# NVlabs/DREAM

Hardware: AMD Instinct MI355X
Metric: frames/s DREAM-vgg-q 400x400 b=128 inference (higher is better)
Workload: dtype f32

## Files before the change

### dream_amd/csrc/conv_first.hip

```cpp
#include <dream_cdna4.h>
#include "common.h"
#include "../../include/dream_hip.h"

namespace {
constexpr int FT = 16;
constexpr int FPW = FT + 4;
constexpr int FPH = FT + 2;
constexpr int FMAXC = 4;
constexpr int FPAIRS = FPH - 1;
constexpr int FPLANE = FPAIRS * FPW * 2;


struct FirstParams {
    const float *x;
    const float *w;
    const float *bias;
    float *y;
    unsigned *amax_out;
    int B, H, W, Cin, Cout;
    int tiles_x, tiles_y;
    int relu;
};

__global__ void __launch_bounds__(256) conv3x3_first_kernel(const FirstParams p) {
    DREAM_DYNAMIC_LDS(float, smem);
    const int tid = threadIdx.x, lane = tid & 63, wave = wave_index();
    int t = blockIdx.x;
    const int tix = t % p.tiles_x;
    t /= p.tiles_x;
    const int tiy = t % p.tiles_y;
    const int b = t / p.tiles_y;
    const int y0 = tiy * FT, x0 = tix * FT;
    const int cout = blockIdx.y * 64 + lane;

    const int npatch = p.Cin * FPH * FPW;
    for (int idx = tid; idx < npatch; idx += 256) {
        const int c = idx / (FPH * FPW);
        const int rem = idx - c * (FPH * FPW);
        const int py = rem / FPW, px = rem - py * FPW;
        const int gy = y0 - 1 + py, gx = x0 - 1 + px;
        float v = 0.0f;
        if (px < FT + 2 && gy >= 0 && gy < p.H && gx >= 0 && gx < p.W)
            v = p.x[(((size_t)b * p.Cin + c) * p.H + gy) * p.W + gx];
        if (py < FPAIRS) smem[c * FPLANE + (py * FPW + px) * 2] = v;
        if (py > 0) smem[c * FPLANE + ((py - 1) * FPW + px) * 2 + 1] = v;
    }
    float wr[FMAXC * 9];
#pragma unroll
    for (int i = 0; i < FMAXC * 9; ++i) wr[i] = (i < p.Cin * 9) ? p.w[(size_t)cout * p.Cin * 9 + i] : 0.0f;
    const float bv = p.bias ? p.bias[cout] : 0.0f;
    __syncthreads();

    float amax = 0.0f;
    for (int g = 0; g < 8; ++g) {
        const int row = wave * 4 + 2 * (g >> 2), xg = (g & 3) * 4;
        f32x2 acc[4];
#pragma unroll
        for (int i = 0; i < 4; ++i) acc[i] = f32x2{bv, bv};
#pragma unroll
        for (int c = 0; c < FMAXC; ++c) {
            if (c < p.Cin) {
#pragma unroll
                for (int ky = 0; ky < 3; ++ky) {
                    const float *src = smem + c * FPLANE + ((row + ky) * FPW + xg) * 2;
                    const f32x4 q0 = *(const f32x4 *)src, q1 = *(const f32x4 *)(src + 4), q2 = *(const f32x4 *)(src + 8);
                    const f32x2 v[6] = {{q0[0], q0[1]}, {q0[2], q0[3]}, {q1[0], q1[1]}, {q1[2], q1[3]}, {q2[0], q2[1]}, {q2[2], q2[3]}};
#pragma unroll
                    for (int kx = 0; kx < 3; ++kx) {
                        const float wv = wr[c * 9 + ky * 3 + kx];
                        const f32x2 w2 = {wv, wv};
#pragma unroll
                        for (int i = 0; i < 4; ++i) acc[i] = __builtin_elementwise_fma(v[i + kx], w2, acc[i]);
                    }
                }
            }
        }
        if (p.relu) {
#pragma unroll
            for (int i = 0; i < 4; ++i) acc[i] = f32x2{fmaxf(acc[i][0], 0.0f), fmaxf(acc[i][1], 0.0f)};
        }
        const int ox = x0 + xg;
#pragma unroll
        for (int h = 0; h < 2; ++h) {
            const int oy = y0 + row + h;
            if (oy < p.H) {
                float *dst = p.y + (((size_t)b * p.H + oy) * p.W + ox) * p.Cout + cout;
#pragma unroll
                for (int i = 0; i < 4; ++i)
                    if (ox + i < p.W) { dst[(size_t)i * p.Cout] = acc[i][h]; amax = fmaxf(amax, fabsf(acc[i][h])); }
            }
        }
    }
    if (p.amax_out != nullptr) publish_amax(p.amax_out, amax);
}
}

static int first_impl(const float *x_nchw, const float *w_oihw, const float *bias, float *y_nhwc, int B, int H, int W,
                      int Cin, int Cout, int relu, void *stream, unsigned *amax_out) {
    DREAM_REQUIRE(x_nchw && w_oihw && y_nhwc, "null pointer");
    DREAM_REQUIRE(B > 0 && H > 0 && W > 0, "bad shape");
    DREAM_REQUIRE(Cin >= 1 && Cin <= FMAXC, "first conv supports Cin <= %d (got %d)", FMAXC, Cin);
    DREAM_REQUIRE(Cout % 64 == 0, "first conv needs Cout %% 64 == 0 (got %d)", Cout);
    FirstParams p;
    p.x = x_nchw; p.w = w_oihw; p.bias = bias; p.y = y_nhwc; p.amax_out = amax_out;
    p.B = B; p.H = H; p.W = W; p.Cin = Cin; p.Cout = Cout; p.relu = relu;
    p.tiles_x = ceil_div(W, FT); p.tiles_y = ceil_div(H, FT);
    const size_t lds = (size_t)Cin * FPLANE * sizeof(float);
    const dim3 grid((unsigned)((size_t)B * p.tiles_x * p.tiles_y), (unsigned)(Cout / 64));
    hipLaunchKernelGGL(conv3x3_first_kernel, grid, dim3(256), lds, (hipStream_t)stream, p);
    DREAM_LAUNCH_OK();
    return 0;
}

extern "C" int dream_conv3x3_first_nchw_f32(const float *x_nchw, const float *w_oihw, const float *bias,
                                            float *y_nhwc, int B, int H, int W, int Cin, int Cout,
                                            int relu, void *stream) {
    return first_impl(x_nchw, w_oihw, bias, y_nhwc, B, H, W, Cin, Cout, relu, stream, nullptr);
}
extern "C" int dream_conv3x3_first_nchw_amax_f32(const float *x_nchw, const float *w_oihw, const float *bias,
                                                 float *y_nhwc, unsigned *amax_out, int B, int H, int W, int Cin,
                                                 int Cout, int relu, void *stream) {
    return first_impl(x_nchw, w_oihw, bias, y_nhwc, B, H, W, Cin, Cout, relu, stream, amax_out);
}
```

### dream_amd/csrc/conv_wino4.hip

```cpp
#include <type_traits>
#include <stdlib.h>
#include <dream_cdna4.h>
#include "common.h"
#include "pack_device.h"
#include "../../include/dream_hip.h"

#ifndef DREAM_W4_DIAG
#define DREAM_W4_DIAG 0
#endif
#ifndef DREAM_W4_STORE
#define DREAM_W4_STORE buffer_store_f32
#endif
#ifndef DREAM_W4_MIDBARRIER
#define DREAM_W4_MIDBARRIER 0
#endif
#ifndef DREAM_W4_STAGGER_N
#define DREAM_W4_STAGGER_N 0
#define DREAM_W4_STAGGER_PCT 0
#endif
#ifndef DREAM_W4_WAUX
#define DREAM_W4_WAUX 0
#endif
#ifndef DREAM_W4_XAUX
#define DREAM_W4_XAUX 0
#endif
#ifndef DREAM_W4_STAG_LX
#define DREAM_W4_STAG_LX 0
#endif
#ifndef DREAM_W4_RUNNING_WOFF
#define DREAM_W4_RUNNING_WOFF 1
#endif
#ifndef DREAM_W4_SETPRIO
#define DREAM_W4_SETPRIO 0
#endif

namespace {

struct Wino4Params {
    const float *x;
    const float *u;
    const float *scale;
    const float *shift;
    const float *residual;
    float *y;
    float *y_full;
    int B, H, W, Cin, Cout, CoutPad;
    int TY, TX;
    int ntiles;
    int nblk, blk_per_xcd;
    unsigned long long magic_tpi, magic_tx;
    int flags;
    int out_scale, out_oy, out_ox;
    int in_scale, in_oy, in_ox;
    int stagger_n, stagger_unit;
    int ymap;
};

constexpr int W4T = 16;
constexpr int W4P = 36;
#ifndef DREAM_W4_RING
#define DREAM_W4_RING 8
#endif
#ifndef DREAM_W4_NARROW_RING
#define DREAM_W4_NARROW_RING 18
#endif
#ifndef DREAM_W4_PAT_RING
#define DREAM_W4_PAT_RING 10
#endif
#ifndef DREAM_W4_PAT_S1OFF
#define DREAM_W4_PAT_S1OFF 8
#endif


template <bool NARROW>
struct W4Cfg {
    static constexpr int NW = NARROW ? 4 : 8;
    static constexpr int K = NARROW ? 8 : 16;
    static constexpr int Q = K / 4;
    static constexpr int KS = K / 4;
    static constexpr int PAD = 16 * NW;
    static constexpr int VPS = NARROW ? W4T * K : W4T * K + 16;
    static constexpr int VB = W4P * VPS;
    static constexpr int SROW = NARROW ? 14 : 25;
    static constexpr int QS = NARROW ? 7 : 6;
    static constexpr int SB = W4T * 6 * SROW * 4;
    static constexpr int RING = NARROW ? DREAM_W4_NARROW_RING : DREAM_W4_RING;
    static constexpr int AHEAD = RING - 2;
    static_assert(72 % RING == 0, "the weight ring must divide two chunks' positions");
    using vec = std::conditional_t<NARROW, f32x2, f32x4>;
};
template <bool NARROW>
DREAM_DEVICE int v4_slot(int q, int t) { return NARROW ? q ^ ((t >> 3) & 1) : q ^ ((t >> 2) & 2); }

DREAM_DEVICE f32x4 fma4(float c, f32x4 a, f32x4 b) {
    f32x4 r;
#pragma unroll
    for (int k = 0; k < 4; ++k) r[k] = __builtin_fmaf(c, a[k], b[k]);
    return r;
}

DREAM_DEVICE f32x4 sub4(f32x4 y, f32x4 x) { return pk_sub4(y, x); }
DREAM_DEVICE f32x4 bt_row(int j, const f32x4 *d) {
    switch (j) {
        case 0: return fma4(-2.0f, d[2], fma4(1.5f, sub4(d[3], d[1]), d[0] + d[4]));
        case 1: return fma4(2.5f, d[3], fma4(0.5f, d[2], sub4(d[4], d[1])));
        case 2: return fma4(0.5f, d[3], fma4(-2.5f, d[2], d[4] + d[1]));
        case 3: return fma4(2.0f, sub4(d[3], d[1]), sub4(d[4], d[2]));
        case 4: return fma4(-0.5f, sub4(d[3], d[1]), sub4(d[4], d[2]));
        default: return fma4(-2.0f, d[3], fma4(1.5f, sub4(d[4], d[2]), d[1] + d[5]));
    }
}

DREAM_DEVICE constexpr bool pat4_row_active(int pat, int i) { return pat == 0 || (((pat - 1) >> 1) == 0 ? i <= 4 : i >= 1); }
DREAM_DEVICE constexpr bool pat4_col_active(int pat, int j) { return pat == 0 || (((pat - 1) & 1) == 0 ? j <= 4 : j >= 1); }
DREAM_DEVICE constexpr bool pat4_active(int pat, int pp) { return pat4_row_active(pat, pp / 6) && pat4_col_active(pat, pp % 6); }
DREAM_DEVICE constexpr int pat4_count(int pat) { return pat == 0 ? 36 : 25; }
struct Pat4Table { int pos[36]; };
constexpr Pat4Table pat4_table(int pat) {
    Pat4Table t = {};
    int n = 0;
    for (int pp = 0; pp < 36; ++pp)
        if (pat4_active(pat, pp)) t.pos[n++] = pp;
    return t;
}
template <int PAT>
struct Pat4 { static constexpr Pat4Table table = pat4_table(PAT); };
#define pat4_pos(PAT, k) (Pat4<PAT>::table.pos[k])

template <int MODE, bool NARROW, int PAT = 0>
__global__ void __launch_bounds__(64 * W4Cfg<NARROW>::NW, 2) conv_wino4_kernel(const Wino4Params p) {
    using C = W4Cfg<NARROW>;
    using vec = typename C::vec;
    constexpr int W4K = C::K, W4NW = C::NW, V4PS = C::VPS, V4B = C::VB, S4ROW = C::SROW;
    constexpr int NPOS = pat4_count(PAT);
    constexpr int W4_RING = PAT ? DREAM_W4_PAT_RING : C::RING, W4_AHEAD = W4_RING - 2;
    static_assert((2 * NPOS) % W4_RING == 0, "the weight ring must divide two chunks' positions");
    DREAM_DYNAMIC_LDS(float, sV);
    const int tid = threadIdx.x;
    const int lane = tid & 63;
    const int wave = wave_index();
    const int item_id = wave * 48 + (lane < 48 ? lane : lane - 16);

    const int xcd = (int)(blockIdx.x & 7), J = (int)(gridDim.x >> 3);
    const int part = p.ymap ? xcd / p.ymap : xcd;
    const int blk_hi = (part + 1) * p.blk_per_xcd;
    const int blk_end = blk_hi < p.nblk ? blk_hi : p.nblk;
    int tb = part * p.blk_per_xcd + (int)(blockIdx.x >> 3);
    if (tb >= blk_end) return;
    const int n0 = (p.ymap ? xcd % p.ymap : (int)blockIdx.y) * (16 * W4NW);
    if (p.stagger_n > 1) {
        const unsigned w = blockIdx.x + blockIdx.y * gridDim.x;
        const int naps = (int)((w * 2654435761u >> 16) % (unsigned)p.stagger_n) * p.stagger_unit;
        for (int i = 0; i < naps; ++i) __builtin_amdgcn_s_sleep(127);
    }
    const int tiles_per_img = p.TY * p.TX;
    const int Si = PAT ? p.in_scale : 1;
    const size_t img_floats = (size_t)(Si * p.H) * (Si * p.W) * p.Cin;

    const int q1 = item_id % C::Q, r1 = (item_id / C::Q) % 6, t1 = (item_id / C::Q) / 6;
    const int s1_off = ((t1 * 6 + r1) * S4ROW + C::QS * q1) * 4;
    const int q2 = item_id % C::Q;
    const int j2 = NARROW ? (item_id >> 3) % 6 : (item_id >> 2) % 6;
    const int t2 = NARROW ? 4 * (item_id / 48) + ((item_id >> 1) & 3) : (item_id >> 2) / 6;
    const int s2_off = ((t2 * 6) * S4ROW + C::QS * q2 + j2) * 4;
    const int v2_off = j2 * V4PS + t2 * W4K + 4 * v4_slot<NARROW>(q2, t2);

    unsigned goff0;
    int item1 = t1 | (r1 << 8) | (q1 << 16);
    auto plan_item = [&](int tile0, int b0) {
        asm volatile("" : "+v"(item1));
        const int t = item1 & 255, r = (item1 >> 8) & 255, q = (item1 >> 16) & 255;
        const int tau = tile0 + t;
        const bool tv = tau < p.ntiles;
        const int b = div_magic40(tau, p.magic_tpi), rem = tau - b * tiles_per_img;
        const int ty = div_magic40(rem, p.magic_tx), tx = rem - ty * p.TX;
        const int gy = 4 * ty - 1 + r, x0 = 4 * tx - 1;
        const bool rok = tv & ((unsigned)gy < (unsigned)p.H);
        goff0 = PAT ? (unsigned)(((((b - b0) * Si * p.H + Si * gy + p.in_oy) * (Si * p.W) + Si * x0 + p.in_ox) * p.Cin + 4 * q) * 4)
                    : (unsigned)(((((b - b0) * p.H + gy) * p.W + x0) * p.Cin + 4 * q) * 4);
        item1 &= 0xffffff;
#pragma unroll
        for (int c = 0; c < 6; ++c) item1 |= (rok & ((unsigned)(x0 + c) < (unsigned)p.W)) ? (1 << (24 + c)) : 0;
    };
    const unsigned px_in = (unsigned)(Si * p.Cin * 4);
    auto item_offset = [&](int c) {
        if (DREAM_W4_DIAG & 16) {
            unsigned o = BUFFER_OOB;
            asm volatile("" : "+v"(o));
            return o;
        }
        return (item1 >> (24 + c)) & 1 ? goff0 + (unsigned)c * px_in : BUFFER_OOB;
    };
    auto block_tile0 = [&](int blk) { return blk < blk_end ? blk * W4T : p.ntiles; };
    auto block_xbuf = [&](int b0) {
        return make_buffer(p.x + (size_t)b0 * img_floats, ((size_t)(p.B - b0) * img_floats) * sizeof(float));
    };

    const int lt = lane & 15, lg = lane >> 4;
    const int a_off = NARROW ? lt * W4K + 4 * v4_slot<NARROW>(lg >> 1, lt) + 2 * (lg & 1) : lt * W4K + 4 * v4_slot<NARROW>(lg, lt);
    const unsigned b_lane = (unsigned)(((wave * 16 + lt) * W4K + C::KS * lg) * 4);
    const unsigned u_pos_stride = (unsigned)(p.CoutPad * W4K * 4);
    const BufferRsrc ubuf = make_buffer(p.u + (size_t)n0 * W4K, ((size_t)((p.Cin / W4K) * W4P + C::AHEAD) * p.CoutPad - (size_t)n0) * W4K * sizeof(float));

    f32x4 acc[W4P];
    const int nchunks = p.Cin / W4K;
    if (DREAM_W4_SETPRIO && wave >= W4NW / 2) __builtin_amdgcn_s_setprio(1);

    vec bq[W4_RING];
    auto load_u = [&](unsigned soff) {
        if constexpr (NARROW) return buffer_load_x2(ubuf, b_lane, soff);
        else return buffer_load_x4_aux<DREAM_W4_WAUX>(ubuf, b_lane, soff);
    };
#pragma unroll
    for (int k = 0; k < W4_AHEAD; ++k) bq[k] = load_u((unsigned)pat4_pos(PAT, k) * u_pos_stride);
    unsigned woff = (unsigned)W4_AHEAD * u_pos_stride;
    DREAM_OPAQUE_SGPR(woff);

    f32x4 *const sV4 = (f32x4 *)sV;
    vec *const sVa = (vec *)sV;
    int vrd[2], vwr[2], s1p = (2 * V4B + s1_off) / 4, s2p = (2 * V4B + s2_off) / 4;
#pragma unroll
    for (int h = 0; h < 2; ++h) {
        vrd[h] = (h * V4B + a_off) / C::KS;
        vwr[h] = (h * V4B + v2_off) / 4;
        asm volatile("" : "+v"(vrd[h]), "+v"(vwr[h]));
    }
    asm volatile("" : "+v"(s1p), "+v"(s2p));
    f32x4 d[6];
    auto pass1_piece = [&](int j) { sV4[s1p + j] = bt_row(j, d); };
    auto pass2_read = [&](int r) { d[r] = sV4[s2p + r * S4ROW]; };
    auto pass2_piece = [&](int i, int h) { if (pat4_row_active(PAT, i)) sV4[vwr[h] + i * (6 * V4PS / 4)] = bt_row(i, d); };

    vec a[2][2];
    auto read_a = [&](int set, int k, int h) {
        const int p0 = pat4_pos(PAT, k), p1 = pat4_pos(PAT, k + 1 < NPOS ? k + 1 : k);
        if constexpr (NARROW) {
            a[set][0] = lds_read_unmerged(sVa + vrd[h] + p0 * V4PS / C::KS);
            a[set][1] = lds_read_unmerged(sVa + vrd[h] + p1 * V4PS / C::KS);
        } else {
            a[set][0] = sVa[vrd[h] + p0 * V4PS / C::KS];
            if (k + 1 < NPOS) a[set][1] = sVa[vrd[h] + p1 * V4PS / C::KS];
        }
    };

    int tile0 = block_tile0(tb);
    int b0 = div_magic40(tile0, p.magic_tpi);
    BufferRsrc xbuf = block_xbuf(b0);
    plan_item(tile0, b0);
#pragma unroll
    for (int c = 0; c < 6; ++c) d[c] = buffer_load_x4(xbuf, item_offset(c), 0u);
#pragma unroll
    for (int j = 0; j < 6; ++j) pass1_piece(j);
    __syncthreads();
#pragma unroll
    for (int r = 0; r < 6; ++r) pass2_read(r);
#pragma unroll
    for (int i = 0; i < 6; ++i) pass2_piece(i, 0);
    __syncthreads();

    auto chunk = [&](auto ph_tag, auto stag_tag, bool last, int c, int tile0n, int b0n) __attribute__((always_inline)) {
        constexpr int PH = decltype(ph_tag)::value;
        constexpr int STAG = decltype(stag_tag)::value;
#ifndef DREAM_W4_S1
#define DREAM_W4_S1 10
#define DREAM_W4_S2 13
#define DREAM_W4_LX 3
#endif
        constexpr int NSLOT = (NPOS + 1) / 2;
        constexpr int S1 = PAT ? NSLOT - DREAM_W4_PAT_S1OFF : DREAM_W4_S1, S2 = PAT ? S1 + 3 : DREAM_W4_S2;
        constexpr int LX = PAT ? 1 : DREAM_W4_LX;
        constexpr int LX0 = STAG ? DREAM_W4_STAG_LX : 0;
        static_assert(LX0 + LX <= S1, "the patch loads must be issued before pass 1");
        const unsigned coff = last ? 0u : (unsigned)((c + 1) * W4K * 4);
        const int cnext = last ? 0 : (c + 1) * W4P;
        if (PH == 1 && last) xbuf = block_xbuf(b0n);
        read_a(0, 0, PH);
        __builtin_amdgcn_sched_barrier(0);
#pragma unroll
        for (int s = 0; s < NSLOT; ++s) {
            const int k0 = 2 * s;
            const bool two = k0 + 1 < NPOS;
            const int pp = pat4_pos(PAT, k0), pp1 = pat4_pos(PAT, two ? k0 + 1 : k0);
            auto load_b = [&](int half) {
                if ((DREAM_W4_DIAG & 2) || (half && !two)) return;
                const int kn = k0 + half + W4_AHEAD;
                if constexpr (PAT == 0 && DREAM_W4_RUNNING_WOFF && !(DREAM_W4_DIAG & 32)) {
                    if (kn == NPOS && last) woff = 0u;
                    bq[(PH * NPOS + kn) % W4_RING] = load_u(woff);
                    woff += u_pos_stride;
                    DREAM_OPAQUE_SGPR(woff);
                } else {
                    const int spos = kn >= NPOS ? cnext + pat4_pos(PAT, kn - NPOS) : c * W4P + pat4_pos(PAT, kn);
                    bq[(PH * NPOS + kn) % W4_RING] = load_u((DREAM_W4_DIAG & 32) ? 0u : (unsigned)spos * u_pos_stride);
                }
            };
            auto load_x = [&](int col) { if (!(DREAM_W4_DIAG & 1)) d[col] = buffer_load_x4_aux<DREAM_W4_XAUX>(xbuf, item_offset(col), (DREAM_W4_DIAG & 64) ? 0u : coff); };
            auto pair = [&](int r) {
                const int i0 = (PH * NPOS + k0) % W4_RING, i1 = (PH * NPOS + k0 + 1) % W4_RING;
                acc[pp] = mfma_f32_16x16x4(a[s & 1][0][r], bq[i0][r], acc[pp]);
                if (two) acc[pp1] = mfma_f32_16x16x4(a[s & 1][1][r], bq[i1][r], acc[pp1]);
                __builtin_amdgcn_sched_barrier(0);
            };
            auto after = [&](int k) {
                if (k == 0) {
                    load_b(0);
                    if (s + 1 < NSLOT) read_a((s + 1) & 1, k0 + 2, PH);
                    if (PH == 1 && s == 0 && last) plan_item(tile0n, b0n);
                    if (s >= LX0 && s < LX0 + LX) { for (int c2 = 0; c2 < 3 / LX; ++c2) load_x((6 / LX) * (s - LX0) + c2); }
                    if (!(DREAM_W4_DIAG & 8) && s >= S1 && s < S1 + 3) pass1_piece(2 * (s - S1));
                    if (!(DREAM_W4_DIAG & 8) && s == S2) { pass2_read(0); pass2_read(1); }
                    if (!(DREAM_W4_DIAG & 8) && s > S2 && s <= S2 + 3) pass2_piece(2 * (s - S2 - 1), 1 - PH);
                } else if (k == 1) {
                    load_b(1);
                    if (s >= LX0 && s < LX0 + LX) { for (int c2 = 3 / LX; c2 < 6 / LX; ++c2) load_x((6 / LX) * (s - LX0) + c2); }
                    if (!(DREAM_W4_DIAG & 8) && s == S2) { pass2_read(2); pass2_read(3); }
                } else if (k == 2) {
                    if (!(DREAM_W4_DIAG & 8) && s >= S1 && s < S1 + 3) pass1_piece(2 * (s - S1) + 1);
                    if (!(DREAM_W4_DIAG & 8) && s == S2) { pass2_read(4); pass2_read(5); }
                    if (!(DREAM_W4_DIAG & 8) && s > S2 && s <= S2 + 3) pass2_piece(2 * (s - S2 - 1) + 1, 1 - PH);
                }
            };
            if constexpr (NARROW) {
                pair(0);
                after(0);
                after(1);
                pair(1);
                after(2);
            } else {
                pair(0);
                after(0);
                pair(1);
                after(1);
                pair(2);
                after(2);
                pair(3);
            }
            if (s == S1 + 2 && !(DREAM_W4_DIAG & 4)) {
                if (DREAM_W4_MIDBARRIER) __syncthreads();
                __builtin_amdgcn_sched_barrier(0);
            }
        }
        if (!(DREAM_W4_DIAG & 4)) __syncthreads();
    };
    const std::integral_constant<int, 0> ph0{};
    const std::integral_constant<int, 1> ph1{};

    constexpr bool pool = MODE == 1 || MODE == 4, both = MODE == 4, has_res = MODE == 2 || MODE == 3, mask = MODE == 3;
    auto epilogue = [&](auto site_tag, int tile0e, int b0e) {
        if (DREAM_W4_DIAG & 128) {
#pragma unroll
            for (int pp = 0; pp < W4P; ++pp)
                if (pat4_active(PAT, pp)) asm volatile("" :: "v"(acc[pp]));
            return;
        }
        const auto &e = *DREAM_KERNARG_SITE(p, decltype(site_tag)::value);
        const bool relu = (e.flags & DREAM_CONV_RELU) != 0;
        const bool late = MODE == 2 && (e.flags & DREAM_CONV_RES_AFTER_RELU) != 0;
        const int Ho = pool ? e.H / 2 : e.H, Wo = pool ? e.W / 2 : e.W, So = e.out_scale;
        const size_t out_img = (size_t)(So * Ho) * (So * Wo) * e.Cout;
        const unsigned px_b = (unsigned)(So * e.Cout * 4), row_b = (unsigned)(So * So * Wo * e.Cout * 4);
        const int ln = lane_id();
        const int lt = ln & 15, lg = ln >> 4;
        const int col = n0 + wave * 16 + lt;
        const bool cok = col < e.Cout;
        const float sc = (e.scale != nullptr && cok) ? e.scale[col] : 1.0f;
        const float sh = (e.shift != nullptr && cok) ? e.shift[col] : 0.0f;
        const BufferRsrc ybuf = make_buffer(e.y + (size_t)b0e * out_img, (DREAM_W4_DIAG & 256) ? 0 : (size_t)(e.B - b0e) * out_img * sizeof(float));
        const BufferRsrc rbuf = make_buffer(has_res ? e.residual + (size_t)b0e * out_img : e.y,
                                            has_res ? (size_t)(e.B - b0e) * out_img * sizeof(float) : 0);
        const size_t full_img = (size_t)e.H * e.W * e.Cout;
        const unsigned fpx_b = (unsigned)(e.Cout * 4), frow_b = (unsigned)(e.W * e.Cout * 4);
        const BufferRsrc fbuf = make_buffer(both ? e.y_full + (size_t)b0e * full_img : e.y, both ? (size_t)(e.B - b0e) * full_img * sizeof(float) : 0);
        const int tau0 = tile0e + lg * 4;
        int b = div_magic40(tau0, p.magic_tpi);
        const int rem = tau0 - b * tiles_per_img;
        int ty = div_magic40(rem, p.magic_tx), tx = rem - ty * p.TX;
        constexpr int NS = pool ? 2 : 4;
        unsigned basef[2][2];
        int limf[2][2];
        unsigned base4[2][2];
        int lim4[2][2];
        constexpr int FULL = pool ? 0x33 : 0xff;
#pragma unroll
        for (int rp = 0; rp < 2; ++rp)
#pragma unroll
            for (int h = 0; h < 2; ++h) {
                const bool tok = cok & ((tau0 + 2 * rp + h) < p.ntiles);
                const int oy = NS * ty, ox = NS * tx;
                base4[rp][h] = (unsigned)(((((b - b0e) * So * Ho + So * oy + e.out_oy) * (So * Wo) + So * ox + e.out_ox) * e.Cout + col) * 4);
                int m = 0;
#pragma unroll
                for (int i = 0; i < NS; ++i) m |= ((oy + i) < Ho ? 1 << i : 0) | ((ox + i) < Wo ? 16 << i : 0);
                lim4[rp][h] = tok ? m : 0;
                if (both) {
                    basef[rp][h] = (unsigned)(((((b - b0e) * e.H + 4 * ty) * e.W + 4 * tx) * e.Cout + col) * 4);
                    int mf = 0;
#pragma unroll
                    for (int i = 0; i < 4; ++i) mf |= ((4 * ty + i) < e.H ? 1 << i : 0) | ((4 * tx + i) < e.W ? 16 << i : 0);
                    limf[rp][h] = tok ? mf : 0;
                }
                const bool wrap_x = (tx + 1 == p.TX);
                const bool wrap_y = wrap_x & (ty + 1 == p.TY);
                tx = wrap_x ? 0 : tx + 1;
                ty = wrap_y ? 0 : (wrap_x ? ty + 1 : ty);
                b += wrap_y ? 1 : 0;
            }
        auto out_off4 = [&](int rp, int h, int i, int jj) {
            const bool inb = ((lim4[rp][h] >> i) & (lim4[rp][h] >> (4 + jj)) & 1) != 0;
            return inb ? base4[rp][h] + (unsigned)i * row_b + (unsigned)jj * px_b : BUFFER_OOB;
        };
        bool interior4[2];
#pragma unroll
        for (int rp = 0; rp < 2; ++rp) interior4[rp] = wave_all((lim4[rp][0] == FULL) & (lim4[rp][1] == FULL));
        auto load_col0 = [&](int rp, float (&r)[2][4]) {
            if (interior4[rp]) {
#pragma unroll
                for (int h = 0; h < 2; ++h)
#pragma unroll
                    for (int i = 0; i < 4; ++i) r[h][i] = buffer_load_f32(rbuf, base4[rp][h], (unsigned)i * row_b);
            } else {
#pragma unroll
                for (int h = 0; h < 2; ++h)
#pragma unroll
                    for (int i = 0; i < 4; ++i) r[h][i] = buffer_load_f32(rbuf, out_off4(rp, h, i, 0), 0u);
            }
        };
        float r0[2][4], r0n[2][4];
        if (has_res) load_col0(0, r0);
#pragma unroll
        for (int rp = 0; rp < 2; ++rp) {
            const unsigned (&base)[2] = base4[rp];
            auto out_off = [&](int h, int i, int jj) { return out_off4(rp, h, i, jj); };
            const bool all_interior = interior4[rp];
            auto fm = [](float c, f32x2 x, f32x2 y) { return __builtin_elementwise_fma(f32x2{c, c}, x, y); };
            f32x2 sA[6][4];
#pragma unroll
            for (int i = 0; i < 6; ++i) {
                f32x2 m[6];
#pragma unroll
                for (int j = 0; j < 6; ++j)
                    m[j] = pat4_active(PAT, 6 * i + j) ? f32x2{acc[6 * i + j][2 * rp], acc[6 * i + j][2 * rp + 1]} : f32x2{0.0f, 0.0f};
                const f32x2 t1 = pk_sub2(m[1], m[2]), t2 = m[1] + m[2];
                sA[i][0] = (m[0] + t2) + (m[3] + m[4]);
                sA[i][1] = fm(-2.0f, m[4], fm(0.5f, m[3], t1));
                sA[i][2] = fm(4.0f, m[4], fm(0.25f, m[3], t2));
                sA[i][3] = fm(-8.0f, m[4], fm(0.125f, m[3], t1)) + m[5];
            }
            auto finish = [&](float v, float rv) {
                if (has_res) v = mask ? (rv > 0.0f ? v : 0.0f) : (late ? v : v + rv);
                const float vr = fmaxf(v, 0.0f);
                v = relu ? vr : v;
                return (MODE == 2 && late) ? v + rv : v;
            };
            auto columns = [&](auto interior_tag, auto &rcur) {
                constexpr bool interior = decltype(interior_tag)::value;
                auto voff = [&](int h, int i, int j2) { return interior ? base[h] : out_off(h, i, j2); };
                auto soff = [&](int i, int j2) { return interior ? (unsigned)i * row_b + (unsigned)j2 * px_b : 0u; };
                float keep[2][2];
#pragma unroll
                for (int jj = 0; jj < 4; ++jj) {
                    float rnext[2][4];
                    if (has_res && jj == 3 && rp == 0) load_col0(1, r0n);
                    if (has_res && jj + 1 < 4) {
#pragma unroll
                        for (int h = 0; h < 2; ++h)
#pragma unroll
                            for (int i = 0; i < 4; ++i) rnext[h][i] = buffer_load_f32(rbuf, voff(h, i, jj + 1), soff(i, jj + 1));
                    }
                    const f32x2 t1 = pk_sub2(sA[1][jj], sA[2][jj]), t2 = sA[1][jj] + sA[2][jj];
                    f32x2 o4[4];
                    o4[0] = (sA[0][jj] + t2) + (sA[3][jj] + sA[4][jj]);
                    o4[1] = fm(-2.0f, sA[4][jj], fm(0.5f, sA[3][jj], t1));
                    o4[2] = fm(4.0f, sA[4][jj], fm(0.25f, sA[3][jj], t2));
                    o4[3] = fm(-8.0f, sA[4][jj], fm(0.125f, sA[3][jj], t1)) + sA[5][jj];
#pragma unroll
                    for (int i = 0; i < 4; ++i) o4[i] = o4[i] * f32x2{sc, sc} + f32x2{sh, sh};
#pragma unroll
                    for (int h = 0; h < 2; ++h) {
                        if (pool) {
                            float v[4];
#pragma unroll
                            for (int i = 0; i < 4; ++i) v[i] = finish(o4[i][h], 0.0f);
                            if (both) {
#pragma unroll
                                for (int i = 0; i < 4; ++i) {
                                    const bool inb = ((limf[rp][h] >> i) & (limf[rp][h] >> (4 + jj)) & 1) != 0;
                                    DREAM_W4_STORE(fbuf, v[i], inb ? basef[rp][h] + (unsigned)i * frow_b + (unsigned)jj * fpx_b : BUFFER_OOB, 0u);
                                }
                            }
                            if ((jj & 1) == 0) {
                                keep[h][0] = fmaxf(v[0], v[1]);
                                keep[h][1] = fmaxf(v[2], v[3]);
                            } else {
                                DREAM_W4_STORE(ybuf, fmaxf(keep[h][0], fmaxf(v[0], v[1])), voff(h, 0, jj >> 1), soff(0, jj >> 1));
                                DREAM_W4_STORE(ybuf, fmaxf(keep[h][1], fmaxf(v[2], v[3])), voff(h, 1, jj >> 1), soff(1, jj >> 1));
                            }
                        } else {
#pragma unroll
                            for (int i = 0; i < 4; ++i)
                                DREAM_W4_STORE(ybuf, finish(o4[i][h], has_res ? rcur[h][i] : 0.0f), voff(h, i, jj), soff(i, jj));
                        }
                    }
                    if (has_res && jj + 1 < 4) {
#pragma unroll
                        for (int h = 0; h < 2; ++h)
#pragma unroll
                            for (int i = 0; i < 4; ++i) rcur[h][i] = rnext[h][i];
                    }
                }
            };
            if (all_interior) columns(std::true_type{}, r0);
            else columns(std::false_type{}, r0);
            if (has_res && rp == 0) {
#pragma unroll
                for (int h = 0; h < 2; ++h)
#pragma unroll
                    for (int i = 0; i < 4; ++i) r0[h][i] = r0n[h][i];
            }
        }
    };

    auto run_blocks = [&](auto stag_tag) __attribute__((always_inline)) {
        while (true) {
            const int tile0n = block_tile0(tb + J);
            const int b0n = div_magic40(tile0n, p.magic_tpi);
            const f32x4 zero = {0.0f, 0.0f, 0.0f, 0.0f};
#pragma unroll
            for (int pp = 0; pp < W4P; ++pp)
                if (pat4_active(PAT, pp)) acc[pp] = zero;
            for (int c = 0; c < nchunks; c += 2) {
                chunk(ph0, stag_tag, false, c, tile0n, b0n);
                chunk(ph1, stag_tag, c + 2 == nchunks, c + 1, tile0n, b0n);
            }
            epilogue(stag_tag, tile0, b0);
            tb += J;
            if (tb >= blk_end) break;
            tile0 = tile0n;
            b0 = b0n;
        }
    };
    if constexpr (!NARROW && PAT == 0 && DREAM_W4_STAG_LX > 0) {
        if (wave >= W4NW / 2) run_blocks(std::integral_constant<int, 1>{});
        else run_blocks(std::integral_constant<int, 0>{});
    } else {
        run_blocks(std::integral_constant<int, 0>{});
    }
}

static_assert(W4Cfg<false>::K == 16 && W4Cfg<false>::PAD == 128 && W4Cfg<true>::K == 8 && W4Cfg<true>::PAD == 64 && W4P == 36,
              "pack_device.h assumes 16-channel chunks padded to 128 rows / 8-channel chunks padded to 64 rows, 36 positions");
__global__ void __launch_bounds__(256) wino4_pack_kernel(const float *w, float *u, int Cout, int Cin, int mode) {
    dream_pack::winograd4(w, u, Cout, Cin, mode, (int)blockIdx.x, (int)gridDim.x);
}

int g_max_workgroups4 = 0;
int g_stagger_n4 = -1, g_stagger_pct4 = 0;
int g_ymap4 = -1;

bool narrow_rows(int rows) { return rows <= W4Cfg<true>::PAD; }
struct PackShape { int k, rows_pad, ahead; };
PackShape pack_shape(int rows) {
    if (narrow_rows(rows)) return {W4Cfg<true>::K, W4Cfg<true>::PAD, W4Cfg<true>::AHEAD};
    return {W4Cfg<false>::K, (rows + W4Cfg<false>::PAD - 1) / W4Cfg<false>::PAD * W4Cfg<false>::PAD, W4Cfg<false>::AHEAD};
}

template <int MODE, bool NARROW, int PAT = 0>
int launch_wino4(const Wino4Params &p, void *stream) {
    using C = W4Cfg<NARROW>;
    void (*kernel)(const Wino4Params) = conv_wino4_kernel<MODE, NARROW, PAT>;
    const size_t lds = ((size_t)2 * C::VB + C::SB) * sizeof(float);
    if (dream_allow_full_lds((const void *)kernel)) return 2;
    const int ny = (p.Cout + 16 * C::NW - 1) / (16 * C::NW);
    const int resident = g_max_workgroups4 > 0 ? g_max_workgroups4 : (NARROW ? 512 : 256);
    Wino4Params q = p;
    dim3 grid;
    if (g_ymap4 && !NARROW && (ny == 2 || ny == 4) && resident >= 64 && p.nblk >= resident) {
        q.ymap = ny;
        q.blk_per_xcd = (p.nblk + 8 / ny - 1) / (8 / ny);
        grid = dim3((unsigned)(resident / 8 * 8), 1u);
    } else {
        int gx = resident / ny / 8 * 8;
        if (gx < 8) gx = 8;
        if (gx > (p.nblk + 7) / 8 * 8) gx = (p.nblk + 7) / 8 * 8;
        grid = dim3((unsigned)gx, (unsigned)ny);
    }
    hipLaunchKernelGGL(kernel, grid, dim3(64 * C::NW), lds, (hipStream_t)stream, q);
    DREAM_LAUNCH_OK();
    return 0;
}

template <bool NARROW>
int launch_wino4_mode(const Wino4Params &p, int mode, void *stream) {
    switch (mode) {
        case 0: return launch_wino4<0, NARROW>(p, stream);
        case 1: return launch_wino4<1, NARROW>(p, stream);
        case 2: return launch_wino4<2, NARROW>(p, stream);
        case 4: return launch_wino4<4, NARROW>(p, stream);
        default: return launch_wino4<3, NARROW>(p, stream);
    }
}

}

// ... 171 lines not shown
```

### dream_amd/csrc/pack_device.h

```cpp
#pragma once
#include <dream_cdna4.h>

namespace dream_pack {

DREAM_DEVICE void conv1x1(const float *w, float *packed, int Cout, int Cin, int mode, int blk, int nblk) {
    const int rows = mode == 0 ? Cout : Cin, K = mode == 0 ? Cin : Cout;
    const int RowsPad = (rows + 63) / 64 * 64;
    const size_t total = (size_t)(K / 16) * RowsPad * 16;
    for (size_t i = (size_t)blk * 256 + threadIdx.x; i < total; i += (size_t)nblk * 256) {
        const int e = (int)(i & 15);
        const size_t rest = i >> 4;
        const int prow = (int)(rest % RowsPad), t = (int)(rest / RowsPad);
        const int b64 = prow >> 6, n = (prow >> 4) & 3, j = prow & 15;
        const int row = b64 * 64 + 4 * j + n, k = 16 * t + e;
        float v = 0.0f;
        if (row < rows) v = mode == 0 ? w[(size_t)row * Cin + k] : w[(size_t)k * Cin + row];
        packed[i] = v;
    }
}

DREAM_DEVICE void filter3x3(const float *w, int Cin, int rows, int mode, int n, int k, double g[3][3]) {
#pragma unroll
    for (int a = 0; a < 3; ++a)
#pragma unroll
        for (int b = 0; b < 3; ++b) {
            float v = 0.0f;
            if (n < rows) {
                v = (mode == 0) ? w[(((size_t)n * Cin + k) * 3 + a) * 3 + b]
                                : w[(((size_t)k * Cin + n) * 3 + (2 - a)) * 3 + (2 - b)];
            }
            g[a][b] = (double)v;
        }
}

DREAM_DEVICE void filterT3x3(const float *wT, int rows, int cols, int pm, int n, int k, double g[3][3]) {
    const int a = (pm >> 1) & 1, b = pm & 1, bwd = (pm >> 2) & 1;
    const int CoutT = bwd ? cols : rows;
    const int ci = bwd ? n : k, co = bwd ? k : n;
#pragma unroll
    for (int r = 0; r < 3; ++r)
#pragma unroll
        for (int c = 0; c < 3; ++c) {
            int ky, kx;
            bool used;
            if (!bwd) {
                const int dy = r - 1, dx = c - 1;
                ky = a + 1 - 2 * dy; kx = b + 1 - 2 * dx;
                used = (a == 0 ? dy <= 0 : dy >= 0) && (b == 0 ? dx <= 0 : dx >= 0);
            } else {
                ky = a - 1 + 2 * r; kx = b - 1 + 2 * c;
                used = (a == 0 ? r >= 1 : r <= 1) && (b == 0 ? c >= 1 : c <= 1);
            }
            float v = 0.0f;
            if (used && n < rows) v = wT[(((size_t)ci * CoutT + co) * 4 + ky) * 4 + kx];
            g[r][c] = (double)v;
        }
}

template <bool CONVT = false>
DREAM_DEVICE void winograd2(const float *w, float *u, int Cout, int Cin, int mode, int blk, int nblk) {
    const int rows = CONVT ? Cout : (mode == 0 ? Cout : Cin), cols = CONVT ? Cin : (mode == 0 ? Cin : Cout);
    const int RowsPad = (rows + 127) / 128 * 128;
    const size_t total = (size_t)(cols / 16) * RowsPad * 16;
    for (size_t i = (size_t)blk * 256 + threadIdx.x; i < total; i += (size_t)nblk * 256) {
        const int kk = (int)(i % 16);
        const size_t rest = i / 16;
        const int n = (int)(rest % RowsPad);
        const int ch = (int)(rest / RowsPad);
        double g[3][3];
        if (CONVT) filterT3x3(w, rows, cols, mode, n, ch * 16 + kk, g);
        else filter3x3(w, Cin, rows, mode, n, ch * 16 + kk, g);
        double t[4][3];
#pragma unroll
        for (int b = 0; b < 3; ++b) {
            t[0][b] = g[0][b];
            t[1][b] = 0.5 * (g[0][b] + g[1][b] + g[2][b]);
            t[2][b] = 0.5 * (g[0][b] - g[1][b] + g[2][b]);
            t[3][b] = g[2][b];
        }
#pragma unroll
        for (int a = 0; a < 4; ++a) {
            const double rr[4] = {t[a][0], 0.5 * (t[a][0] + t[a][1] + t[a][2]), 0.5 * (t[a][0] - t[a][1] + t[a][2]), t[a][2]};
#pragma unroll
            for (int b = 0; b < 4; ++b)
                u[(((size_t)ch * 16 + (a * 4 + b)) * RowsPad + n) * 16 + kk] = (float)(a == 3 ? -rr[b] : rr[b]);
        }
    }
}

template <bool CONVT = false>
DREAM_DEVICE void winograd4(const float *w, float *u, int Cout, int Cin, int mode, int blk, int nblk) {
    const double G[6][3] = {{1.0, 0.0, 0.0},
                            {1.0 / 3.0, 1.0 / 3.0, 1.0 / 3.0},
                            {-1.0 / 3.0, 1.0 / 3.0, -1.0 / 3.0},
                            {-16.0 / 15.0, -8.0 / 15.0, -4.0 / 15.0},
                            {1.0 / 15.0, -2.0 / 15.0, 4.0 / 15.0},
                            {0.0, 0.0, 1.0}};
    const int rows = CONVT ? Cout : (mode == 0 ? Cout : Cin), cols = CONVT ? Cin : (mode == 0 ? Cin : Cout);
    const int K = rows <= 64 ? 8 : 16;
    const int RowsPad = rows <= 64 ? 64 : (rows + 127) / 128 * 128;
    const size_t total = (size_t)(cols / K) * RowsPad * K;
    for (size_t i = (size_t)blk * 256 + threadIdx.x; i < total; i += (size_t)nblk * 256) {
        const int kk = (int)(i % K);
        const size_t rest = i / K;
        const int n = (int)(rest % RowsPad);
        const int ch = (int)(rest / RowsPad);
        double g[3][3];
        if (CONVT) filterT3x3(w, rows, cols, mode, n, ch * K + kk, g);
        else filter3x3(w, Cin, rows, mode, n, ch * K + kk, g);
        double t[6][3];
#pragma unroll
        for (int a = 0; a < 6; ++a)
#pragma unroll
            for (int b = 0; b < 3; ++b) t[a][b] = G[a][0] * g[0][b] + G[a][1] * g[1][b] + G[a][2] * g[2][b];
#pragma unroll
        for (int a = 0; a < 6; ++a)
#pragma unroll
            for (int b = 0; b < 6; ++b) {
                const double v = t[a][0] * G[b][0] + t[a][1] * G[b][1] + t[a][2] * G[b][2];
                u[(((size_t)ch * 36 + (a * 6 + b)) * RowsPad + n) * K + kk] = (float)v;
            }
    }
}

}
```

Before: 2600.

## Persistent double-buffered first conv and paired narrow Winograd weight loads

The first 3x3 conv becomes a persistent, Cin-templated kernel. Its grid is sized to the resident workgroup count, and it double-buffers input tiles in LDS so the next tile's global loads overlap the current tile's compute. Each lane now computes 4 output channels × 4 pixels and writes them with vectorized buffer stores, which raises arithmetic per LDS read. Separately, the narrow Winograd-4 weight transform interleaves pairs of positions so the main kernel fetches two positions' B operands with one x4 load instead of two x2 loads, at the cost of a new weight layout tied to a compile-time flag.

```diff
diff --git a/dream_amd/csrc/conv_first.hip b/dream_amd/csrc/conv_first.hip
--- a/dream_amd/csrc/conv_first.hip
+++ b/dream_amd/csrc/conv_first.hip
@@ -1,3 +1,4 @@
+#include <stdlib.h>
 #include <dream_cdna4.h>
 #include "common.h"
 #include "../../include/dream_hip.h"
@@ -7,9 +8,9 @@
 constexpr int FPW = FT + 4;
 constexpr int FPH = FT + 2;
 constexpr int FMAXC = 4;
-constexpr int FPAIRS = FPH - 1;
-constexpr int FPLANE = FPAIRS * FPW * 2;
-
+constexpr int FPLANE = FPH * FPW;
+constexpr int FIRST_WG_PER_CU = 3;
+constexpr int FIRST_CUS = 256;
 
 struct FirstParams {
     const float *x;
@@ -18,80 +19,136 @@
     float *y;
     unsigned *amax_out;
     int B, H, W, Cin, Cout;
-    int tiles_x, tiles_y;
+    int tiles_x, tiles_y, ntiles;
     int relu;
 };
 
-__global__ void __launch_bounds__(256) conv3x3_first_kernel(const FirstParams p) {
+template <int CIN>
+__global__ void __launch_bounds__(256, CIN <= 3 ? 3 : 2) conv3x3_first_kernel(const FirstParams p) {
     DREAM_DYNAMIC_LDS(float, smem);
+    constexpr int NPATCH = CIN * FPLANE;
     const int tid = threadIdx.x, lane = tid & 63, wave = wave_index();
+    const int cq = lane & 15, lg = lane >> 4;
+    const int cout = blockIdx.y * 64 + 4 * cq;
     int t = blockIdx.x;
-    const int tix = t % p.tiles_x;
-    t /= p.tiles_x;
-    const int tiy = t % p.tiles_y;
-    const int b = t / p.tiles_y;
-    const int y0 = tiy * FT, x0 = tix * FT;
-    const int cout = blockIdx.y * 64 + lane;
+    if (t >= p.ntiles) return;
 
-    const int npatch = p.Cin * FPH * FPW;
-    for (int idx = tid; idx < npatch; idx += 256) {
-        const int c = idx / (FPH * FPW);
-        const int rem = idx - c * (FPH * FPW);
-        const int py = rem / FPW, px = rem - py * FPW;
-        const int gy = y0 - 1 + py, gx = x0 - 1 + px;
-        float v = 0.0f;
-        if (px < FT + 2 && gy >= 0 && gy < p.H && gx >= 0 && gx < p.W)
-            v = p.x[(((size_t)b * p.Cin + c) * p.H + gy) * p.W + gx];
-        if (py < FPAIRS) smem[c * FPLANE + (py * FPW + px) * 2] = v;
-        if (py > 0) smem[c * FPLANE + ((py - 1) * FPW + px) * 2 + 1] = v;
-    }
-    float wr[FMAXC * 9];
+    float wq[CIN * 9][4];
 #pragma unroll
-    for (int i = 0; i < FMAXC * 9; ++i) wr[i] = (i < p.Cin * 9) ? p.w[(size_t)cout * p.Cin * 9 + i] : 0.0f;
-    const float bv = p.bias ? p.bias[cout] : 0.0f;
-    __syncthreads();
+    for (int i = 0; i < CIN * 9; ++i)
+#pragma unroll
+        for (int j = 0; j < 4; ++j) wq[i][j] = p.w[(size_t)(cout + j) * (CIN * 9) + i];
+    f32x4 bv = {0.0f, 0.0f, 0.0f, 0.0f};
+    if (p.bias)
+#pragma unroll
+        for (int j = 0; j < 4; ++j) bv[j] = p.bias[cout + j];
+
+    constexpr int SROWS = 12, SN = SROWS * FPW, NSTG = (CIN * FPH + SROWS - 1) / SROWS;
+    struct Tile { int b, y0, x0; };
+    auto decode = [&](int tt) {
+        const int tix = tt % p.tiles_x;
+        tt /= p.tiles_x;
+        const int tiy = tt % p.tiles_y;
+        return Tile{tt / p.tiles_y, tiy * FT, tix * FT};
+    };
+    auto stage_load = [&](const Tile &tl, float (&v)[NSTG]) {
+        const BufferRsrc img = make_buffer(p.x + (size_t)tl.b * CIN * p.H * p.W, (size_t)CIN * p.H * p.W * sizeof(float));
+        int ti = tid;
+        asm volatile("" : "+v"(ti));
+        const int ry = ti / FPW, px = ti - ry * FPW;
+        const int gx = (ti < SN && px < FT + 2) ? tl.x0 - 1 + px : -1;
+        const bool xok = (unsigned)gx < (unsigned)p.W;
+#pragma unroll
+        for (int k = 0; k < NSTG; ++k) {
+            const int R = ry + SROWS * k, c0 = (SROWS * k) / FPH;
+            const int c = c0 + (R >= FPH * (c0 + 1) ? 1 : 0), gy = tl.y0 - 1 + R - FPH * c;
+            const bool ok = xok && R < CIN * FPH && (unsigned)gy < (unsigned)p.H;
+            v[k] = buffer_load_f32(img, ok ? (unsigned)((c * p.H + gy) * p.W + gx) * 4u : BUFFER_OOB, 0u);
+        }
+    };
+    auto stage_write = [&](float *buf, const float (&v)[NSTG]) {
+#pragma unroll
+        for (int k = 0; k < NSTG; ++k)
+            if (tid < SN && tid + SN * k < NPATCH) buf[tid + SN * k] = v[k];
+    };
 
     float amax = 0.0f;
-    for (int g = 0; g < 8; ++g) {
-        const int row = wave * 4 + 2 * (g >> 2), xg = (g & 3) * 4;
-        f32x2 acc[4];
+    const unsigned px_b = (unsigned)p.Cout * 4u, voff = (unsigned)(4 * lg) * px_b + (unsigned)cout * 4u;
+    auto compute = [&](const Tile &tl, const float *buf) {
+#pragma unroll 1
+        for (int r = 0; r < 4; ++r) {
+            const int row = wave * 4 + r, oy = tl.y0 + row;
+            if (oy >= p.H) break;
+            f32x4 acc[4];
 #pragma unroll
-        for (int i = 0; i < 4; ++i) acc[i] = f32x2{bv, bv};
+            for (int i = 0; i < 4; ++i) acc[i] = bv;
+            const float *src = buf + row * FPW + 4 * lg;
+            f32x4 q0 = *(const f32x4 *)src;
+            f32x2 q1 = *(const f32x2 *)(src + 4);
 #pragma unroll
-        for (int c = 0; c < FMAXC; ++c) {
-            if (c < p.Cin) {
+            for (int g = 0; g < CIN * 3; ++g) {
+                const float v[6] = {q0[0], q0[1], q0[2], q0[3], q1[0], q1[1]};
+                if (g + 1 < CIN * 3) {
+                    const float *nsrc = src + ((g + 1) / 3) * FPLANE + ((g + 1) % 3) * FPW;
+                    q0 = *(const f32x4 *)nsrc;
+                    q1 = *(const f32x2 *)(nsrc + 4);
+                }
+                __builtin_amdgcn_sched_barrier(0);
 #pragma unroll
-                for (int ky = 0; ky < 3; ++ky) {
-                    const float *src = smem + c * FPLANE + ((row + ky) * FPW + xg) * 2;
-                    const f32x4 q0 = *(const f32x4 *)src, q1 = *(const f32x4 *)(src + 4), q2 = *(const f32x4 *)(src + 8);
-                    const f32x2 v[6] = {{q0[0], q0[1]}, {q0[2], q0[3]}, {q1[0], q1[1]}, {q1[2], q1[3]}, {q2[0], q2[1]}, {q2[2], q2[3]}};
+                for (int kx = 0; kx < 3; ++kx)
 #pragma unroll
-                    for (int kx = 0; kx < 3; ++kx) {
-                        const float wv = wr[c * 9 + ky * 3 + kx];
-                        const f32x2 w2 = {wv, wv};
+                    for (int i = 0; i < 4; ++i)
 #pragma unroll
-                        for (int i = 0; i < 4; ++i) acc[i] = __builtin_elementwise_fma(v[i + kx], w2, acc[i]);
-                    }
+                        for (int j = 0; j < 4; ++j) acc[i][j] = __builtin_fmaf(v[i + kx], wq[g * 3 + kx][j], acc[i][j]);
+                __builtin_amdgcn_sched_barrier(0);
+            }
+            if (p.relu) {
+#pragma unroll
+                for (int i = 0; i < 4; ++i)
+#pragma unroll
+                    for (int j = 0; j < 4; ++j) acc[i][j] = fmaxf(acc[i][j], 0.0f);
+            }
+            const int npx = p.W - tl.x0 < FT ? p.W - tl.x0 : FT;
+            const BufferRsrc yrow = make_buffer(p.y + (((size_t)tl.b * p.H + oy) * p.W + tl.x0) * p.Cout, (size_t)npx * p.Cout * sizeof(float));
+#pragma unroll
+            for (int i = 0; i < 4; ++i) buffer_store_x4(yrow, acc[i], voff + (unsigned)i * px_b, 0u);
+            if (p.amax_out != nullptr) {
+#pragma unroll
+                for (int i = 0; i < 4; ++i) {
+                    const float m = fmaxf(fmaxf(fabsf(acc[i][0]), fabsf(acc[i][1])), fmaxf(fabsf(acc[i][2]), fabsf(acc[i][3])));
+                    amax = fmaxf(amax, 4 * lg + i < npx ? m : 0.0f);
                 }
             }
         }
-        if (p.relu) {
-#pragma unroll
-            for (int i = 0; i < 4; ++i) acc[i] = f32x2{fmaxf(acc[i][0], 0.0f), fmaxf(acc[i][1], 0.0f)};
-        }
-        const int ox = x0 + xg;
-#pragma unroll
-        for (int h = 0; h < 2; ++h) {
-            const int oy = y0 + row + h;
-            if (oy < p.H) {
-                float *dst = p.y + (((size_t)b * p.H + oy) * p.W + ox) * p.Cout + cout;
-#pragma unroll
-                for (int i = 0; i < 4; ++i)
-                    if (ox + i < p.W) { dst[(size_t)i * p.Cout] = acc[i][h]; amax = fmaxf(amax, fabsf(acc[i][h])); }
-            }
-        }
+    };
+
+    Tile cur = decode(t);
+    float sv[NSTG];
+    stage_load(cur, sv);
+    stage_write(smem, sv);
+    __syncthreads();
+    int ib = 0;
+    while (true) {
+        const int tn = t + (int)gridDim.x;
+        const bool more = tn < p.ntiles;
+        const Tile nxt = decode(more ? tn : t);
+        if (more) stage_load(nxt, sv);
+        compute(cur, smem + ib * NPATCH);
+        if (!more) break;
+        ib ^= 1;
+        stage_write(smem + ib * NPATCH, sv);
+        __syncthreads();
+        t = tn;
+        cur = nxt;
     }
     if (p.amax_out != nullptr) publish_amax(p.amax_out, amax);
+}
+
+template <int CIN>
+void launch_first(const FirstParams &p, int gx, void *stream) {
+    void (*kernel)(const FirstParams) = conv3x3_first_kernel<CIN>;
+    const size_t lds = (size_t)2 * CIN * FPLANE * sizeof(float);
+    hipLaunchKernelGGL(kernel, dim3((unsigned)gx, (unsigned)(p.Cout / 64)), dim3(256), lds, (hipStream_t)stream, p);
 }
 }
 
@@ -101,13 +158,28 @@
     DREAM_REQUIRE(B > 0 && H > 0 && W > 0, "bad shape");
     DREAM_REQUIRE(Cin >= 1 && Cin <= FMAXC, "first conv supports Cin <= %d (got %d)", FMAXC, Cin);
     DREAM_REQUIRE(Cout % 64 == 0, "first conv needs Cout %% 64 == 0 (got %d)", Cout);
+    DREAM_REQUIRE((size_t)Cin * H * W * sizeof(float) < ((size_t)1 << 31), "first conv: image too large for 32-bit offsets");
     FirstParams p;
     p.x = x_nchw; p.w = w_oihw; p.bias = bias; p.y = y_nhwc; p.amax_out = amax_out;
     p.B = B; p.H = H; p.W = W; p.Cin = Cin; p.Cout = Cout; p.relu = relu;
     p.tiles_x = ceil_div(W, FT); p.tiles_y = ceil_div(H, FT);
-    const size_t lds = (size_t)Cin * FPLANE * sizeof(float);
-    const dim3 grid((unsigned)((size_t)B * p.tiles_x * p.tiles_y), (unsigned)(Cout / 64));
-    hipLaunchKernelGGL(conv3x3_first_kernel, grid, dim3(256), lds, (hipStream_t)stream, p);
+    const size_t ntiles = (size_t)B * p.tiles_x * p.tiles_y;
+    DREAM_REQUIRE(ntiles < ((size_t)1 << 31), "first conv: too many tiles");
+    p.ntiles = (int)ntiles;
+    int resident = FIRST_CUS * FIRST_WG_PER_CU;
+    if (const char *e = getenv("DREAM_FIRST_MAX_WORKGROUPS")) {
+        const int cap = atoi(e);
+        if (cap > 0) resident = cap;
+    }
+    int gx = resident / (Cout / 64);
+    if (gx < 1) gx = 1;
+    if (gx > p.ntiles) gx = p.ntiles;
+    switch (Cin) {
+        case 1: launch_first<1>(p, gx, stream); break;
+        case 2: launch_first<2>(p, gx, stream); break;
+        case 3: launch_first<3>(p, gx, stream); break;
+        default: launch_first<4>(p, gx, stream); break;
+    }
     DREAM_LAUNCH_OK();
     return 0;
 }
diff --git a/dream_amd/csrc/conv_wino4.hip b/dream_amd/csrc/conv_wino4.hip
--- a/dream_amd/csrc/conv_wino4.hip
+++ b/dream_amd/csrc/conv_wino4.hip
@@ -87,6 +87,8 @@
     static constexpr int RING = NARROW ? DREAM_W4_NARROW_RING : DREAM_W4_RING;
     static constexpr int AHEAD = RING - 2;
     static_assert(72 % RING == 0, "the weight ring must divide two chunks' positions");
+    static constexpr bool PAIRS = NARROW && DREAM_W4_NARROW_PAIRS;
+    static_assert(!PAIRS || RING % 2 == 0, "a ring of whole pairs");
     using vec = std::conditional_t<NARROW, f32x2, f32x4>;
 };
 template <bool NARROW>
@@ -198,7 +200,7 @@
 
     const int lt = lane & 15, lg = lane >> 4;
     const int a_off = NARROW ? lt * W4K + 4 * v4_slot<NARROW>(lg >> 1, lt) + 2 * (lg & 1) : lt * W4K + 4 * v4_slot<NARROW>(lg, lt);
-    const unsigned b_lane = (unsigned)(((wave * 16 + lt) * W4K + C::KS * lg) * 4);
+    const unsigned b_lane = C::PAIRS ? (unsigned)(((wave * 16 + lt) * 16 + 4 * lg) * 4) : (unsigned)(((wave * 16 + lt) * W4K + C::KS * lg) * 4);
     const unsigned u_pos_stride = (unsigned)(p.CoutPad * W4K * 4);
     const BufferRsrc ubuf = make_buffer(p.u + (size_t)n0 * W4K, ((size_t)((p.Cin / W4K) * W4P + C::AHEAD) * p.CoutPad - (size_t)n0) * W4K * sizeof(float));
 
@@ -206,13 +208,15 @@
     const int nchunks = p.Cin / W4K;
     if (DREAM_W4_SETPRIO && wave >= W4NW / 2) __builtin_amdgcn_s_setprio(1);
 
-    vec bq[W4_RING];
+    constexpr int BSTEP = C::PAIRS ? 2 : 1;
+    std::conditional_t<C::PAIRS, f32x4, vec> bq[W4_RING / BSTEP];
     auto load_u = [&](unsigned soff) {
-        if constexpr (NARROW) return buffer_load_x2(ubuf, b_lane, soff);
+        if constexpr (C::PAIRS) return buffer_load_x4(ubuf, b_lane, soff);
+        else if constexpr (NARROW) return buffer_load_x2(ubuf, b_lane, soff);
         else return buffer_load_x4_aux<DREAM_W4_WAUX>(ubuf, b_lane, soff);
     };
 #pragma unroll
-    for (int k = 0; k < W4_AHEAD; ++k) bq[k] = load_u((unsigned)pat4_pos(PAT, k) * u_pos_stride);
+    for (int k = 0; k < W4_AHEAD; k += BSTEP) bq[k / BSTEP] = load_u((unsigned)pat4_pos(PAT, k) * u_pos_stride);
     unsigned woff = (unsigned)W4_AHEAD * u_pos_stride;
     DREAM_OPAQUE_SGPR(woff);
 
@@ -283,22 +287,28 @@
             const int pp = pat4_pos(PAT, k0), pp1 = pat4_pos(PAT, two ? k0 + 1 : k0);
             auto load_b = [&](int half) {
                 if ((DREAM_W4_DIAG & 2) || (half && !two)) return;
+                if (C::PAIRS && half) return;
                 const int kn = k0 + half + W4_AHEAD;
                 if constexpr (PAT == 0 && DREAM_W4_RUNNING_WOFF && !(DREAM_W4_DIAG & 32)) {
                     if (kn == NPOS && last) woff = 0u;
-                    bq[(PH * NPOS + kn) % W4_RING] = load_u(woff);
-                    woff += u_pos_stride;
+                    bq[(PH * NPOS + kn) % W4_RING / BSTEP] = load_u(woff);
+                    woff += BSTEP * u_pos_stride;
                     DREAM_OPAQUE_SGPR(woff);
                 } else {
                     const int spos = kn >= NPOS ? cnext + pat4_pos(PAT, kn - NPOS) : c * W4P + pat4_pos(PAT, kn);
-                    bq[(PH * NPOS + kn) % W4_RING] = load_u((DREAM_W4_DIAG & 32) ? 0u : (unsigned)spos * u_pos_stride);
+                    bq[(PH * NPOS + kn) % W4_RING / BSTEP] = load_u((DREAM_W4_DIAG & 32) ? 0u : (unsigned)spos * u_pos_stride);
                 }
             };
             auto load_x = [&](int col) { if (!(DREAM_W4_DIAG & 1)) d[col] = buffer_load_x4_aux<DREAM_W4_XAUX>(xbuf, item_offset(col), (DREAM_W4_DIAG & 64) ? 0u : coff); };
             auto pair = [&](int r) {
                 const int i0 = (PH * NPOS + k0) % W4_RING, i1 = (PH * NPOS + k0 + 1) % W4_RING;
-                acc[pp] = mfma_f32_16x16x4(a[s & 1][0][r], bq[i0][r], acc[pp]);
-                if (two) acc[pp1] = mfma_f32_16x16x4(a[s & 1][1][r], bq[i1][r], acc[pp1]);
+                if constexpr (C::PAIRS) {
+                    acc[pp] = mfma_f32_16x16x4(a[s & 1][0][r], bq[i0 / 2][r], acc[pp]);
+                    acc[pp1] = mfma_f32_16x16x4(a[s & 1][1][r], bq[i0 / 2][2 + r], acc[pp1]);
+                } else {
+                    acc[pp] = mfma_f32_16x16x4(a[s & 1][0][r], bq[i0][r], acc[pp]);
+                    if (two) acc[pp1] = mfma_f32_16x16x4(a[s & 1][1][r], bq[i1][r], acc[pp1]);
+                }
                 __builtin_amdgcn_sched_barrier(0);
             };
             auto after = [&](int k) {
diff --git a/dream_amd/csrc/pack_device.h b/dream_amd/csrc/pack_device.h
--- a/dream_amd/csrc/pack_device.h
+++ b/dream_amd/csrc/pack_device.h
@@ -88,6 +88,9 @@
     }
 }
 
+#ifndef DREAM_W4_NARROW_PAIRS
+#define DREAM_W4_NARROW_PAIRS 1
+#endif
 template <bool CONVT = false>
 DREAM_DEVICE void winograd4(const float *w, float *u, int Cout, int Cin, int mode, int blk, int nblk) {
     const double G[6][3] = {{1.0, 0.0, 0.0},
@@ -118,7 +121,11 @@
 #pragma unroll
             for (int b = 0; b < 6; ++b) {
                 const double v = t[a][0] * G[b][0] + t[a][1] * G[b][1] + t[a][2] * G[b][2];
-                u[(((size_t)ch * 36 + (a * 6 + b)) * RowsPad + n) * K + kk] = (float)v;
+                const int pp = a * 6 + b;
+                if (DREAM_W4_NARROW_PAIRS && K == 8)
+                    u[(((((size_t)ch * 18 + pp / 2) * RowsPad + n) * 4 + kk / 2) * 2 + (pp & 1)) * 2 + (kk & 1)] = (float)v;
+                else
+                    u[(((size_t)ch * 36 + pp) * RowsPad + n) * K + kk] = (float)v;
             }
     }
 }
```

Result: faster. 2629, median of 6 (+1.1%).
